# serval-uni-lu/moeva2-ijcai22-replication

Measured on AMD Instinct MI355X. Metric: candidate fitness evals/sec (whole node) + attack wall-clock per 1k states, higher is better.
Workload: dtype f64; 1 GPU; rq1.botnet.static; states=387, states_per_gpu=387, pop_size=203, n_offsprings=100, n_gen=1000, norm=2, history=reduced, classifier_dtype=f32 (MFMA), crossover=two_point, genes_stored=312, schedule=per-phase kernel chain

## Files before the change

include/moeva_mi355x.h:

```cpp
#ifndef MOEVA_MI355X_H
#define MOEVA_MI355X_H

#include <stdint.h>

#ifdef __cplusplus
extern "C" {
#endif

enum {
  MV_OK = 0,
  MV_ERR_ARG = 1,
  MV_ERR_HIP = 2,
  MV_ERR_STATE = 3,
};

enum { MV_GENE_REAL = 0, MV_GENE_INT = 1, MV_GENE_OHE = 2 };

enum {
  MV_OP_DIFF = 1,
  MV_OP_RATIO_SAFE = 2,
  MV_OP_ABS_SUMDIFF = 3,
  MV_OP_LCLD_INSTALL = 4,
  MV_OP_LCLD_TERM = 5,
  MV_OP_ABS_RATIO = 6,
// ... 84 lines not shown
  const double* ml_scale;
  const double* ml_min;
  int32_t norm;
} mv_objcalc_desc;
typedef struct mv_objcalc mv_objcalc;
int mv_objcalc_create(int32_t device, const mv_objcalc_desc* desc, mv_objcalc** out);
void mv_objcalc_destroy(mv_objcalc* o);
int mv_objcalc_run(mv_objcalc* o, mv_engine* constraints, mv_mlp* classifier, int32_t B,
                   int32_t n, const double* x_init, const double* x, int32_t minimize_class,
                   double* obj, int32_t* range_bad, void* stream);
int mv_objcalc_score(mv_objcalc* o, int32_t B, int32_t n, const double* x_init, const double* x,
                     const double* G, int32_t C, const double* proba, int32_t n_out,
                     int32_t minimize_class, double* obj, int32_t* range_bad, void* stream);
typedef struct mv_attack_params {
  int32_t n_gen;
  int32_t pop_size;
  int32_t n_offsprings;
  uint64_t seed;
  int32_t n_ref;
  const double* ref_points;
  double mu;
  int32_t history;
} mv_attack_params;

int mv_attack_run(mv_engine* e, const mv_attack_params* params, void* stream);
int mv_set_attack_mode(mv_engine* e, int32_t mode);
int mv_set_state_streams(mv_engine* e, int32_t enabled, int64_t first_state);
int mv_set_mlp_precision(mv_engine* e, int32_t bf16);
int mv_get_attack_time(mv_engine* e, double* ms, int32_t* whole);
int mv_attack_population(mv_engine* e, double* genes, double* F, void* stream);
int mv_attack_front(mv_engine* e, uint8_t* front, int32_t* offsets, double* X, double* Fx,
                    void* stream);
int mv_attack_history(mv_engine* e, double* hist, void* stream);
int mv_get_stored_genes(mv_engine* e, int32_t* stored, int32_t* n_stored);
int mv_gene_layout(mv_engine* e, int32_t B, const double* x_init, const double* xl,
                   const double* xu, int32_t* stored, int32_t* n_stored);
int mv_set_gene_layout(mv_engine* e, const int32_t* stored, int32_t V);
int mv_set_profiling(mv_engine* e, int32_t enabled);
int mv_get_kernel_times(mv_engine* e, double* vary_ms, double* mlp_ms, double* survive_ms,
                        int32_t* n_generations);
int mv_get_phase_times(mv_engine* e, double* ms, int32_t* n_generations);
int mv_get_row_kernel(mv_engine* e, int32_t* kind);
int mv_get_mlp_kernel(mv_engine* e, int32_t* kind);

int mv_debug_checks(int32_t* record, int32_t* compiled);
int mv_debug_survival_dump(double* out);

int mv_det_pow(int64_t n, const double* x, const double* y, double* out);

typedef struct mv_pgd_desc {
  int32_t D;
  const double* ml_scale;
  const double* ml_min;
  const int32_t* mutable_mask;
  int32_t C;
  const int32_t* op_code;
  const int32_t* op_arg;
  const double* op_karg;
  int32_t n_pool;
  const int32_t* idx_pool;
  int32_t n_ohe;
  const int32_t* ohe_offsets;
  const int32_t* ohe_feats;
  int32_t repair_install[4];
  double tol;
} mv_pgd_desc;
// ... 28 lines not shown
```

moeva2-ijcai22-replication_amd/csrc/api.cpp:

```cpp
#include <hip/hip_runtime.h>

#include <cmath>
#include <cstdio>
#include <cstdlib>
#include <algorithm>
#include <numeric>
#include <cstring>
#include <string>
#include <vector>

#include "../../include/moeva_mi355x.h"
#include "check.h"
#include "detmath.h"
#include "engine.h"
#include "kernels.h"
#include "pgd.h"
#include "rowops.h"

using namespace mv;

namespace mv {
thread_local hipEvent_t g_ev_start = nullptr, g_ev_stop = nullptr;
}

// ... 82 lines not shown
  DProblem p{};
  std::vector<void*> prob_allocs;
  bool compact = false;
  std::vector<int> stored;
  std::vector<int> layout_req;
  DProblem pc{};
  std::vector<void*> compact_allocs;
  DStates sc{};
  double* genes0c = nullptr;
  std::vector<void*> cstate_allocs;
  const DProblem& ap() const { return compact ? pc : p; }
  const DStates& as() const { return compact ? sc : s; }
  double* ag0() const { return compact ? genes0c : genes0; }
  float* W1full = nullptr;
  float* b1 = nullptr;
  int H1 = 0;
  int B = 0;
  std::vector<void*> state_allocs;
  DStates s{};
  double* genes0 = nullptr;
  std::vector<void*> attack_allocs;
  int P = 0, O = 0, S = 0, n_gen = 0, R = 0, hist_mode = 0, hist_w = 0, hist_rows = 0;
  double* pool = nullptr;
  double* poolF = nullptr;
  int* pop_slot = nullptr;
  int* free_slot = nullptr;
  int* parents = nullptr;
  bool has_plan = false;
  int4* plan_hdr = nullptr;
  int* plan_mw = nullptr;
  double* plan_mu = nullptr;
  double *ideal = nullptr, *worst = nullptr, *extreme = nullptr;
  int* has_ext = nullptr;
  double* ref = nullptr;
  std::vector<double> ref_host;
  double* hist = nullptr;
  unsigned char* front_scr = nullptr;
  int* off_scr = nullptr;
  bool attack_ready = false;
  bool has_model = false;
  long long* d_phase = nullptr;
  long long* d_gphase = nullptr;
  bool gphase_mlp = false;
  size_t gphase_n = 0;
  unsigned long long* dom_g = nullptr;
  size_t dom_stride = 0;
  float* xml = nullptr;
  size_t xml_cap = 0;
  hipError_t ensure_xml(size_t rows) {
    const size_t need = rows * (size_t)p.Dm4;
    if (need <= xml_cap) return hipSuccess;
    if (xml) (void)hipFree(xml);
    xml = nullptr;
    xml_cap = 0;
    hipError_t e = dalloc(&xml, need);
    if (e == hipSuccess) xml_cap = need;
    return e;
  }
  hipStream_t streams[MAX_GROUPS] = {};
  hipEvent_t ev_fork = nullptr;
  hipEvent_t ev_join[MAX_GROUPS] = {};
  hipError_t ensure_streams(int n) {
    hipError_t err = hipSuccess;
    if (!ev_fork) err = hipEventCreateWithFlags(&ev_fork, hipEventDisableTiming);
    for (int q = 1; q < n && err == hipSuccess; ++q) {
      if (!streams[q]) err = hipStreamCreateWithFlags(&streams[q], hipStreamNonBlocking);
// ... 280 lines not shown

int mv_engine_create(int32_t device, const mv_problem_desc* pd, const mv_model_desc* md,
                     mv_engine** out) {
  if (!pd || !out) return fail(MV_ERR_ARG, "null argument");
  *out = nullptr;
  const int D = pd->D, V = pd->V, Dm = pd->Dm, C = pd->C;
  if (D <= 0 || V <= 0 || Dm <= 0 || C < 0) return fail(MV_ERR_ARG, "bad problem sizes");
  if (pd->D * 4 * 8 > 160 * 1024) return fail(MV_ERR_ARG, "D too large");
  if (md && (md->n_layers < 2 || md->n_layers > MAX_LAYERS))
    return fail(MV_ERR_ARG, "classifier must have 2..6 Dense layers");
  if (md) {
    if (md->dims[0] != D) return fail(MV_ERR_ARG, "model input width != D");
    for (int l = 1; l < md->n_layers; ++l)
      if (md->dims[l] % 16 != 0 || md->dims[l] > 512 || md->dims[l] <= 0)
        return fail(MV_ERR_ARG, "hidden widths must be multiples of 16 and <= 512");
    if (md->dims[md->n_layers] < 2 || md->dims[md->n_layers] > 8)
      return fail(MV_ERR_ARG, "softmax output width must be 2..8");
  }
  for (int j = 1; j < Dm; ++j)
    if (pd->mut_feats[j] <= pd->mut_feats[j - 1]) return fail(MV_ERR_ARG, "mut_feats not ascending");
  int ns[2] = {0, 0};
  for (int g = 0; g < V; ++g) {
    const int k = pd->gene_kind[g];
    if (k < 0 || k > 2) return fail(MV_ERR_ARG, "bad gene kind");
    const int sub = ns[k == MV_GENE_REAL ? 0 : 1]++;
    if (pd->gene_feat[g] < 0 || pd->gene_feat[g] > 0x7FFF || sub > 0x7FFF)
      return fail(MV_ERR_ARG, "feature/gene index too large for the packed gene table");
  }
  if (V > VARY_MAX_V || ((Dm + 15) & ~15) > VARY_MAX_V)
    return fail(MV_ERR_ARG, "genetic length / mutable features must be <= 1024");
  HIPCHK(hipSetDevice(device));
  mv_engine* e = new mv_engine();
  e->device = device;
  HostProblem& h = e->hp;
  h.D = D;
  h.V = V;
  h.Dm = Dm;
  h.C = C;
  h.n_ohe = pd->n_ohe;
  h.n_pool = pd->n_pool;
  h.norm = pd->norm;
  h.scale_obj = pd->scale_objectives;
  h.tol = pd->tol;
  h.kind.assign(pd->gene_kind, pd->gene_kind + V);
  h.feat.assign(pd->gene_feat, pd->gene_feat + V);
  h.ohe_off.assign(pd->n_ohe + 1, 0);
  if (pd->n_ohe > 0) std::memcpy(h.ohe_off.data(), pd->ohe_offsets, (pd->n_ohe + 1) * sizeof(int));
  const int n_ohe_feats = pd->n_ohe > 0 ? pd->ohe_offsets[pd->n_ohe] : 0;
  h.ohe_feats.assign(pd->ohe_feats, pd->ohe_feats + n_ohe_feats);
  h.mut.assign(pd->mut_feats, pd->mut_feats + Dm);
  h.op_code.assign(pd->op_code, pd->op_code + C);
  h.op_arg.assign(pd->op_arg, pd->op_arg + (size_t)C * 4);
  h.op_k.assign(pd->op_karg, pd->op_karg + (size_t)C * 2);
  h.pool.assign(pd->idx_pool, pd->idx_pool + pd->n_pool);
  h.mls.assign(D, 1.0);
  h.mlm.assign(D, 0.0);
  if (pd->ml_scale) std::memcpy(h.mls.data(), pd->ml_scale, D * sizeof(double));
  if (pd->ml_min) std::memcpy(h.mlm.data(), pd->ml_min, D * sizeof(double));
  if (md) {
    e->has_model = true;
    HostModel& m = e->hm;
    m.n_layers = md->n_layers;
    for (int l = 0; l <= md->n_layers; ++l) m.dims[l] = md->dims[l];
    for (int l = 0; l < md->n_layers; ++l) {
      m.W[l].assign(md->W[l], md->W[l] + (size_t)md->dims[l] * md->dims[l + 1]);
      m.b[l].assign(md->b[l], md->b[l] + md->dims[l + 1]);
// ... 371 lines not shown
    auto A = [&](auto** dst, size_t n) {
      if (err != hipSuccess) return;
      err = dalloc(dst, n);
      if (err == hipSuccess) e->attack_allocs.push_back((void*)*dst);
    };
    e->d_gphase = nullptr;
    e->gphase_n = 0;
    e->front_scr = nullptr;
    e->off_scr = nullptr;
    A(&e->pool, (size_t)B * S * V);
    A(&e->poolF, (size_t)B * S * 3);
    A(&e->pop_slot, (size_t)B * P);
    A(&e->free_slot, (size_t)B * O);
    A(&e->parents, (size_t)B * O);
    e->plan_hdr = nullptr;
    e->plan_mw = nullptr;
    e->plan_mu = nullptr;
    if (use_plan) {
      A(&e->plan_hdr, (size_t)B * O);
      A(&e->plan_mw, (size_t)B * O * PLAN_MUT);
      A(&e->plan_mu, (size_t)B * O * PLAN_MUT);
    }
    e->has_plan = use_plan;
    e->dom_g = nullptr;
    e->dom_stride = 0;
    if (S > SURV_NLDS) {
      e->dom_stride = (size_t)S * ((S + 63) / 64);
      A(&e->dom_g, (size_t)B * e->dom_stride);
    }
    A(&e->ideal, (size_t)B * 3);
    A(&e->worst, (size_t)B * 3);
    A(&e->extreme, (size_t)B * 9);
    A(&e->has_ext, (size_t)B);
    A(&e->ref, (size_t)R * 3);
    if (prm->history) A(&e->hist, (size_t)B * hist_rows * hist_w);
    if (err != hipSuccess)
      return fail(MV_ERR_HIP, std::string("attack alloc: ") + hipGetErrorString(err));
    e->P = P;
    e->O = O;
    e->S = S;
    e->R = R;
    e->n_gen = G;
    e->hist_mode = prm->history;
    e->hist_w = hist_w;
    e->hist_rows = hist_rows;
    e->attack_ready = true;
  }
  if (realloc || e->ref_host.size() != (size_t)R * 3 ||
      std::memcmp(e->ref_host.data(), prm->ref_points, (size_t)R * 3 * sizeof(double)) != 0) {
    HIPCHK(hipDeviceSynchronize());
    e->ref_host.assign(prm->ref_points, prm->ref_points + (size_t)R * 3);
    HIPCHK(hipMemcpy(e->ref, e->ref_host.data(), (size_t)R * 3 * sizeof(double),
                     hipMemcpyHostToDevice));
  }
  hipLaunchKernelGGL(k_fill_d, dim3(64), dim3(256), 0, stream, e->ideal, (size_t)B * 3,
                     (double)INFINITY);
  hipLaunchKernelGGL(k_fill_d, dim3(64), dim3(256), 0, stream, e->worst, (size_t)B * 3,
                     (double)-INFINITY);
  hipLaunchKernelGGL(k_fill_i, dim3(64), dim3(256), 0, stream, e->has_ext, (size_t)B, 0);
  HIPCHK(hipGetLastError());
  HIPCHK(launch_init_pool(B, P, O, V, S, e->ag0(), e->pool, e->pop_slot, e->free_slot, stream));
  HIPCHK(e->ensure_xml((size_t)B * (P > O ? P : O)));
  int ngrp = B / 64;
  ngrp = ngrp > 4 ? 4 : ngrp;
  if (const char* g = std::getenv("MV_GROUPS")) ngrp = std::atoi(g);
  if (e->profiling) ngrp = 1;
  ngrp = ngrp < 1 ? 1 : (ngrp > MAX_GROUPS ? MAX_GROUPS : (ngrp > B ? B : ngrp));
  HIPCHK(e->ensure_streams(ngrp));
  hipStream_t gs[MAX_GROUPS];
  int gb0[MAX_GROUPS + 1];
  for (int q = 0; q <= ngrp; ++q) gb0[q] = (int)((long long)B * q / ngrp);
  gs[0] = stream;
  if (ngrp > 1) HIPCHK(hipEventRecord(e->ev_fork, stream));
  for (int q = 1; q < ngrp; ++q) {
    gs[q] = e->streams[q];
    HIPCHK(hipStreamWaitEvent(gs[q], e->ev_fork, 0));
  }
  const int H1 = e->H1, D = ap.D;
  const unsigned sbb = vary_offsets(ap).sb;
  const size_t Dm4 = ap.Dm4;
  auto group_rows = [&](RowsArgs r, int q, int n_per_state) {
    const size_t b0 = gb0[q];
    r.s.B = gb0[q + 1] - gb0[q];
    r.s.x_init += b0 * D;
    r.s.gl += b0 * V;
    r.s.gu += b0 * V;
    r.s.sblob += b0 * sbb;
    r.s.bias1 += b0 * H1;
    r.s.min_class += b0;
    r.total = r.s.B * n_per_state;
    r.key0 += (uint32_t)b0;
    if (r.genes_in) r.genes_in += b0 * r.in_rows * V;
    if (r.genes_out) r.genes_out += b0 * r.out_rows * V;
    if (r.parents) r.parents += b0 * O;
    if (r.out_map) r.out_map += b0 * r.n;
    if (r.plan_hdr) {
      r.plan_hdr += b0 * O;
      r.plan_mw += b0 * O * PLAN_MUT;
      r.plan_mu += b0 * O * PLAN_MUT;
    }
    if (r.F) r.F += b0 * r.out_rows * 3;
    if (r.hist) r.hist += b0 * (size_t)r.hist_rows * r.hist_w;
    r.xml += b0 * (size_t)(P > O ? P : O) * Dm4;
    return r;
  };
  auto group_surv = [&](SurvArgs s, int q) {
    const size_t b0 = gb0[q];
    s.F += b0 * S * 3;
    s.pop_slot += b0 * P;
    s.free_slot += b0 * O;
    s.pop_slot_out += b0 * P;
    s.ideal += b0 * 3;
    s.worst += b0 * 3;
    s.extreme += b0 * 9;
    s.has_extreme += b0;
    s.key0 += (uint32_t)b0;
    if (s.parents_out) s.parents_out += b0 * O;
    if (s.phase) s.phase += b0 * 32;
    if (s.dom_g) s.dom_g += b0 * s.dom_stride;
    if (s.plan_hdr) {
      s.plan_hdr += b0 * O;
      s.plan_mw += b0 * O * PLAN_MUT;
      s.plan_mu += b0 * O * PLAN_MUT;
    }
    return s;
  };
  RowsArgs ev = base_rows(e, true);
  ev.n = P;
  ev.mode = 0;
  ev.genes_in = e->pool;
  ev.in_rows = S;
  ev.out_rows = S;
  ev.F = e->poolF;
  ev.hist = prm->history ? e->hist : nullptr;
  ev.hist_rows = hist_rows;
  ev.hist_w = hist_w;
  ev.xml = e->xml;
  SurvArgs sa{};
  sa.n_survive = P;
  sa.P = P;
  sa.O = O;
  sa.F = e->poolF;
  sa.S = S;
  sa.pop_slot = e->pop_slot;
  sa.free_slot = e->free_slot;
  sa.pop_slot_out = e->pop_slot;
  sa.ref = e->ref;
  sa.R = R;
  sa.mu = prm->mu;
  sa.seed = prm->seed;
  sa.state_keys = e->state_keys;
  sa.key0 = e->key0;
  sa.ideal = e->ideal;
  sa.worst = e->worst;
  sa.extreme = e->extreme;
  sa.has_extreme = e->has_ext;
  sa.O_next = O;
  sa.dom_g = e->dom_g;
  sa.dom_stride = e->dom_stride;
  {
    int dev = 0, cus = 0;
    if (hipGetDevice(&dev) != hipSuccess ||
        hipDeviceGetAttribute(&cus, hipDeviceAttributeMultiprocessorCount, dev) != hipSuccess)
      cus = 0;
    (void)hipGetLastError();
    sa.wide = 2 * B <= cus ? 2 : B <= 2 * cus ? 1 : 0;
    if (const char* w = std::getenv("MV_SURV_WIDE")) sa.wide = std::atoi(w);
  }
  if (use_plan) {
    const VaryOff vo = vary_offsets(ap);
    sa.plan_hdr = e->plan_hdr;
    sa.plan_mw = e->plan_mw;
    sa.plan_mu = e->plan_mu;
    sa.geo = (const uint32_t*)(ap.vblob + vo.geo);
    sa.cmap = (const int*)(ap.vblob + vo.cmap);
    sa.ginfo = (const int*)(ap.vblob + vo.ginfo);
    sa.Vr = ap.Vr;
    sa.V = ap.V;
    sa.n_sub0 = ap.n_sub[0];
    sa.n_sub1 = ap.n_sub[1];
    sa.cx_prob = e->cx_prob;
    sa.cx_sbx = e->cx_kind == 1;
  }
  if (std::getenv("MV_SURV_PHASES")) {
    if (!e->d_phase) {
      HIPCHK(hipMalloc((void**)&e->d_phase, (size_t)B * 32 * sizeof(long long)));
      e->attack_allocs.push_back(e->d_phase);
    }
    sa.phase = e->d_phase;
// ... 610 lines not shown
  const DProblem& ap = e->ap();
  const int* cmap = ap.compact ? (const int*)(ap.vblob + vary_offsets(ap).cmap) : nullptr;
  HIPCHK(launch_front(e->B, e->P, ap.V, ap.Vr, e->S, cmap, e->s.gl, e->pop_slot, e->pool,
                      e->poolF, front, offsets, X, Fx, (hipStream_t)stream));
  return MV_OK;
}

int mv_gene_layout(mv_engine* e, int32_t B, const double* x_init, const double* xl,
                   const double* xu, int32_t* stored, int32_t* n_stored) {
  if (!e || B < 0 || (B > 0 && (!x_init || !xl || !xu)) || !stored || !n_stored)
    return fail(MV_ERR_ARG, "bad mv_gene_layout arguments");
  const std::vector<int> keep = B > 0 ? stored_genes(e, B, x_init, xl, xu) : std::vector<int>{};
  for (int g = 0; g < e->hp.V; ++g) stored[g] = keep.empty() ? 1 : 0;
  for (int g : keep) stored[g] = 1;
  *n_stored = keep.empty() ? e->hp.V : (int32_t)keep.size();
  return MV_OK;
}

int mv_set_gene_layout(mv_engine* e, const int32_t* stored, int32_t V) {
  if (!e) return fail(MV_ERR_ARG, "null engine");
  if (!stored) {
    e->layout_req.clear();
    return MV_OK;
  }
  if (V != e->hp.V) return fail(MV_ERR_ARG, "mv_set_gene_layout: V differs from the problem's");
  std::vector<int> keep;
  for (int g = 0; g < V; ++g)
    if (stored[g]) keep.push_back(g);
  if (keep.empty()) return fail(MV_ERR_ARG, "mv_set_gene_layout: no stored gene");
  e->layout_req = keep;
  return MV_OK;
}

int mv_get_stored_genes(mv_engine* e, int32_t* stored, int32_t* n_stored) {
  if (!e || !n_stored) return fail(MV_ERR_ARG, "null argument");
  const DProblem& ap = e->ap();
  *n_stored = ap.V;
  if (stored)
    for (int g = 0; g < ap.Vr; ++g) {
      const auto it = std::lower_bound(e->stored.begin(), e->stored.end(), g);
      stored[g] = !ap.compact || (it != e->stored.end() && *it == g);
    }
  return MV_OK;
}

int mv_attack_history(mv_engine* e, double* hist, void* stream) {
  if (!e || !e->attack_ready || !e->hist_mode) return fail(MV_ERR_STATE, "no history recorded");
  if (!hist) return fail(MV_ERR_ARG, "null hist");
  if (!on_device(hist, e->device))
    return fail(MV_ERR_ARG, "mv_attack_history: hist lives on another device than the engine");
  HIPCHK(hipSetDevice(e->device));
  HIPCHK(hipMemcpyAsync(hist, e->hist, (size_t)e->B * e->hist_rows * e->hist_w * sizeof(double),
                        hipMemcpyDefault, (hipStream_t)stream));
  return MV_OK;
}

struct mv_pgd {
  int device = 0;
  PgdArgs a{};
  std::vector<void*> allocs;
  ~mv_pgd() {
    (void)hipSetDevice(device);
    for (void* x : allocs) (void)hipFree(x);
  }
};

// ... 172 lines not shown
```

moeva2-ijcai22-replication_amd/csrc/engine.h:

```cpp
#pragma once
#include <hip/hip_runtime.h>
#include <stdint.h>

#ifndef MV_CLOCKS
#define MV_CLOCKS 0
#endif

namespace mv {

constexpr int MAX_LAYERS = 6;
constexpr int EVAL_TR = 32;
constexpr int EVAL_T = 256;
#ifndef MV_VARY_T
#define MV_VARY_T 256
#endif
constexpr int VARY_T = MV_VARY_T;
constexpr int VARY_W = VARY_T / 64;
#ifndef MV_CONS_T
#define MV_CONS_T 256
#endif
constexpr int CONS_T = MV_CONS_T;
constexpr int CONS_W = CONS_T / 64;
constexpr int VARY_ROWS_MAX = 32;
constexpr int VARY_MAX_V = 1024;
// ... 123 lines not shown
  double mu;
  uint64_t seed;
  int gen;
  uint32_t stream_key;
  int state_keys;
  uint32_t key0;
  double* ideal;
  double* worst;
  double* extreme;
  int* has_extreme;
  int* survivors;
  int* rank;
  int* order;
  int* n_ranked;
  int* niche;
  double* dist;
  double* nadir;
  int* parents_out;
  int O_next;
  int sel_gen;
  long long* phase;
  unsigned long long* dom_g;
  size_t dom_stride;
  int4* plan_hdr;
  int* plan_mw;
  double* plan_mu;
  const uint32_t* geo;
  const int* cmap;
  const int* ginfo;
  int Vr, V, n_sub0, n_sub1;
  double cx_prob;
  int cx_sbx;
  int wide;
};

struct MlpArgs {
  int n_layers;
  int dims[MAX_LAYERS + 1];
  const float* W[MAX_LAYERS];
  const float* bias[MAX_LAYERS];
  int D4;
  int n;
  const double* x;
  double* proba;
};

struct ObjArgs {
  long total;
  int n;
  int D, C, n_ohe, n_out, cls, norm;
  const double* x;
  const double* x_init;
  const double* mm_scale;
  const double* mm_min;
  const int* ohe_off;
  const int* ohe_feat;
  const double* G;
  const double* proba;
  double* obj;
  int* range_bad;
};

}
```

moeva2-ijcai22-replication_amd/csrc/survival.h:

```cpp
#pragma once
#include <limits.h>

#include "check.h"
#include "draws.h"
#include "engine.h"
#ifdef MV_CHECKS
namespace mv {
static __device__ int g_surv_dump_owner;
static __device__ double g_surv_dump[SURV_DUMP_N];
}
#endif
#include "philox.h"
#include "wave.h"

namespace mv {

constexpr int SURV_TMAX = 1024;
#ifndef MV_ASSOC_UNROLL
#define MV_ASSOC_UNROLL 1
#endif

struct SurvLds {
  double* F;
  const double* ref;
// ... 455 lines not shown
  L.cur = (unsigned long long*)(smem + o.cur);
  L.I = (int*)(smem + o.I);
  L.pos = (int*)(smem + o.pos);
  L.front_of = (int*)(smem + o.front_of);
  L.slot = (int*)(smem + o.slot);
  L.niche = (int*)(smem + o.niche);
  L.memb = (int*)(smem + o.memb);
  L.key = (int*)(smem + o.key);
  L.surv = (int*)(smem + o.surv);
  L.sel = (int*)(smem + o.sel);
  L.fstart = (int*)(smem + o.fstart);
  L.count = (int*)(smem + o.count);
  L.remain = (int*)(smem + o.remain);
  L.csr_off = (int*)(smem + o.csr_off);
  L.csr = (int*)(smem + o.csr);
  L.cand = (int*)(smem + o.cand);
  L.ckey = (int*)(smem + o.ckey);
  L.iscal = (int*)(smem + o.iscal);
  L.sortk = (unsigned long long*)(smem + o.sortk);
  L.perm = (int*)(smem + o.perm);
  L.dmin = (unsigned long long*)(smem + o.dmin);
  L.lround = (int*)(smem + o.lround);
  double* ideal = L.scal;
  double* worst = L.scal + 3;
  double* wpop = L.scal + 6;
  double* wfront = L.wsc + (tid >> 6) * 16;
  double* nadir = wfront + 3;
  double* ext = wfront + 6;
  double* pext = L.scal + 24;
  const int has_ext = a.has_extreme[b] != 0;
  const double pre_ideal = tid < 3 ? a.ideal[(size_t)b * 3 + tid] : 0.0;
  const double pre_worst = tid < 3 ? a.worst[(size_t)b * 3 + tid] : 0.0;
  const bool slot_mode = a.pop_slot != nullptr;
#define PHASE(k) \
  if (MV_CLOCKS && a.phase && tid == 0) a.phase[(size_t)b * 32 + (k)] = clock64();
  PHASE(0)

  for (int m = tid; m < N; m += T) {
    int s = m;
    const double* src;
    if (slot_mode) {
      s = m < a.P ? a.pop_slot[(size_t)b * a.P + m] : a.free_slot[(size_t)b * a.O + (m - a.P)];
      s = MV_IDX(s, a.S, CK_SURV_SLOT);
      src = a.F + ((size_t)b * a.S + s) * 3;
    } else {
      src = a.F + ((size_t)b * N + m) * 3;
    }
    const double f0 = src[0], f1 = src[1], f2 = src[2];
    L.F[m * 3 + 0] = f0;
    L.F[m * 3 + 1] = f1;
    L.F[m * 3 + 2] = f2;
    L.slot[m] = s;
    L.front_of[m] = -1;
    L.sel[m] = 0;
  }
  for (int m = N + tid; m < NW * 64; m += T) {
    L.F[m * 3 + 0] = __builtin_nan("");
    L.F[m * 3 + 1] = __builtin_nan("");
    L.F[m * 3 + 2] = __builtin_nan("");
  }
  if (tid < 9) pext[tid] = a.extreme[(size_t)b * 9 + tid];
  if (tid == 0) L.iscal[14] = 0;
  for (int q = tid; q < NW; q += T) {
    L.ranked[q] = 0ull;
    L.cur[q] = 0ull;
  }
  __syncthreads();
  PHASE(1)

  if (wave == 0) {
    double mn[3], mx[3], wp[3];
    for (int k = 0; k < 3; ++k) {
      mn[k] = __builtin_inf();
      mx[k] = -__builtin_inf();
      wp[k] = -__builtin_inf();
    }
    for (int m = lane; m < N; m += 64)
      for (int k = 0; k < 3; ++k) {
        const double v = L.F[m * 3 + k];
        mn[k] = min_prop(mn[k], v);
        mx[k] = max_prop(mx[k], v);
        wp[k] = max_prop(wp[k], v);
      }
    for (int r = lane; r < R; r += 64)
      for (int k = 0; k < 3; ++k) {
        const double v = L.ref[r * 3 + k];
        mn[k] = min_prop(mn[k], v);
        mx[k] = max_prop(mx[k], v);
      }
    for (int k = 0; k < 3; ++k) {
      mn[k] = wred_min(mn[k]);
      mx[k] = wred_max(mx[k]);
      wp[k] = wred_max(wp[k]);
    }
    if (lane < 3) {
      const int k = lane;
      double vmn = mn[0], vmx = mx[0], vwp = wp[0];
      if (k == 1) {
        vmn = mn[1];
        vmx = mx[1];
        vwp = wp[1];
      } else if (k == 2) {
        vmn = mn[2];
        vmx = mx[2];
        vwp = wp[2];
      }
      ideal[k] = min_prop(pre_ideal, vmn);
      worst[k] = max_prop(pre_worst, vmx);
      wpop[k] = vwp;
    }
  }
  PHASE(11)

  if (NWMAX * 64 > SURV_NLDS) {
    const int n_b = NW * (NW + 1) / 2;
    for (;;) {
      int t = 0;
      if (lane == 0) t = atomicAdd(&L.iscal[14], 1);
      t = __builtin_amdgcn_readfirstlane(t);
      if (t >= n_b) break;
      int qi = 0, rem = t;
      while (rem >= NW - qi) {
        rem -= NW - qi;
        ++qi;
      }
      const int qj = qi + rem;
      const int i = qi * 64 + lane;
      const double fi0 = L.F[i * 3 + 0], fi1 = L.F[i * 3 + 1], fi2 = L.F[i * 3 + 2];
      const int j0 = qj * 64;
      const double* fj = L.F + j0 * 3;
      unsigned mlo = 0u, mhi = 0u;
      unsigned long long acc = 0ull;
      DomRow<0, 64, unsigned long long>::run(fi0, fi1, fi2, fj, mlo, mhi, acc, lane);
      const unsigned long long mine = ((unsigned long long)mhi << 32) | mlo;
      if (j0 + lane < N) L.dom[(size_t)qi * N + j0 + lane] = mine;
      if (qi != qj && i < N) L.dom[(size_t)qj * N + i] = acc;
    }
  } else {
    unsigned short* dom16 = (unsigned short*)L.dom;
    const int n_q = NW * (NW + 1) * 2;
    for (;;) {
      int t = 0;
      if (lane == 0) t = atomicAdd(&L.iscal[14], 1);
      t = __builtin_amdgcn_readfirstlane(t);
      if (t >= n_q) break;
      const int qq = t & 3;
      int qi = 0, rem = t >> 2;
      while (rem >= NW - qi) {
        rem -= NW - qi;
        ++qi;
      }
      const int qj = qi + rem;
      const int i = qi * 64 + lane;
      const double fi0 = L.F[i * 3 + 0], fi1 = L.F[i * 3 + 1], fi2 = L.F[i * 3 + 2];
      const int j0 = qj * 64 + qq * 16;
      const double* fj = L.F + j0 * 3;
      unsigned mlo = 0u, mhi = 0u, acc = 0u;
      DomRow<0, 16, unsigned>::run(fi0, fi1, fi2, fj, mlo, mhi, acc, lane);
      const unsigned long long mine = ((unsigned long long)mhi << 32) | mlo;
      if (lane < 16 && j0 + lane < N)
        L.dom[(size_t)qi * N + j0 + lane] = mine;
      if (qi != qj && i < N) dom16[((size_t)qj * N + i) * 4 + qq] = (unsigned short)acc;
    }
  }
  __syncthreads();
  PHASE(2)

  int* wsum = L.iscal + 16;
  int n0 = block_compact<T>(
      N,
      [&](int j) {
        for (int q = 0; q < NW; ++q)
          if (L.dom[(size_t)q * N + j]) return false;
        return true;
      },
      L.I, 0, wsum);
  for (int k = tid; k < n0; k += T) {
    const int j = L.I[k];
    L.pos[j] = k;
    L.front_of[j] = 0;
    atomicOr(&L.ranked[j >> 6], 1ull << (j & 63));
    atomicOr(&L.cur[j >> 6], 1ull << (j & 63));
  }
  if (tid == 0) {
    L.fstart[0] = 0;
// ... 175 lines not shown
        for (int k = 0; k < 3; ++k) Mc[i][k] = M[i][k];
      bool ok = lu_solve3(Mc, plane);
      double nd[3];
      if (ok) {
        double icp[3];
        for (int k = 0; k < 3; ++k) {
          icp[k] = 1.0 / plane[k];
          nd[k] = ideal[k] + icp[k];
        }
        bool close = true, small = false;
        for (int i = 0; i < 3; ++i) {
          const double mp = (M[i][0] * plane[0] + M[i][1] * plane[1]) + M[i][2] * plane[2];
          close = close && (fabs(mp - 1.0) <= 1e-8 + 1e-5 * 1.0);
          small = small || (icp[i] <= 1e-6);
        }
        if (!close || small) {
          ok = false;
        } else {
          for (int k = 0; k < 3; ++k)
            if (nd[k] > worst[k]) nd[k] = worst[k];
        }
      }
      if (!ok)
        for (int k = 0; k < 3; ++k) nd[k] = wpop[k];
      for (int k = 0; k < 3; ++k) {
        if (nd[k] - ideal[k] <= 1e-6) nd[k] = wfront[k];
        nadir[k] = nd[k];
      }
    }
    wave_sync();
    PHASE(26)
  }
  PHASE(4)

  {
    const double nv = 1.0 / sqrt(3.0);
    const double asp = a.mu * (1.0 / 3.0);
    for (int r = tid; r < RN; r += T) {
      double res[3];
      if (r < R) {
        double l[3];
        for (int k = 0; k < 3; ++k) l[k] = (L.ref[r * 3 + k] - ideal[k]) / (nadir[k] - ideal[k]);
        const double dot = (l[0] * nv + l[1] * nv) + l[2] * nv;
        double inter[3];
        if (fabs(dot) > 1e-6) {
          const double d = ((1.0 * nv + 0.0 * nv) + 0.0 * nv) / dot;
          for (int k = 0; k < 3; ++k) inter[k] = 0.0 + l[k] * d;
        } else {
          const double q0 = l[0] - 1.0, q1 = l[1] - 0.0, q2 = l[2] - 0.0;
          const double t = (q0 * nv + q1 * nv) + q2 * nv;
          for (int k = 0; k < 3; ++k) inter[k] = l[k] - t * nv;
        }
        for (int k = 0; k < 3; ++k) res[k] = asp + (inter[k] - asp);
        if (!(res[0] > 0.0 && res[1] > 0.0 && res[2] > 0.0)) {
          for (int k = 0; k < 3; ++k)
            if (res[k] < 0.0) res[k] = 0.0;
          const double s = (res[0] + res[1]) + res[2];
          for (int k = 0; k < 3; ++k) res[k] = res[k] / s;
        }
      } else {
        for (int k = 0; k < 3; ++k) res[k] = (k == r - R) ? 1.0 : 0.0;
      }
      const double nrm = sqrt((res[0] * res[0] + res[1] * res[1]) + res[2] * res[2]);
      for (int k = 0; k < 3; ++k) L.U[r * 3 + k] = res[k] / nrm;
      L.Uf[r] = make_double4(L.U[r * 3], L.U[r * 3 + 1], L.U[r * 3 + 2], 0.0);
    }
    if (tid == 0) L.iscal[15] = 0;
    __syncthreads();
  }
  PHASE(5)

  {
    double den[3];
    for (int k = 0; k < 3; ++k) {
      den[k] = nadir[k] - ideal[k];
      if (den[k] == 0.0) den[k] = 1e-12;
    }
    const int nh = RN >> 1;
    for (int v = tid; v < 2 * n_ranked; v += T) {
      const int p = v >> 1, hf = v & 1;
      const int jb = hf ? nh : 0;
      const bool odd = hf && (RN & 1);
      const int m = L.I[p];
      double Nn[3];
      for (int k = 0; k < 3; ++k) Nn[k] = (L.F[m * 3 + k] - ideal[k]) / den[k];
      if (Nn[0] == 0.0 && Nn[1] == 0.0 && Nn[2] == 0.0 && !signbit(Nn[0]) && !signbit(Nn[1]) &&
          !signbit(Nn[2])) {
        if (!hf) {
          L.niche[p] = 0;
          L.dist[p] = 0.0;
        }
        continue;
      }
      const double nn = fma(Nn[0], Nn[0], fma(Nn[1], Nn[1], Nn[2] * Nn[2]));
      const double4* Ud = L.Uf;
      auto d2f = [&](int j) {
        const double4 u = Ud[j];
        const double sp = fma(Nn[0], u.x, fma(Nn[1], u.y, Nn[2] * u.z));
        return fma(-sp, sp, nn);
      };
      double b0 = __builtin_inf(), b1 = b0, b2 = b0, b3 = b0;
      const int n4 = nh >> 2;
      if (nn < __builtin_inf()) {
#pragma unroll MV_ASSOC_UNROLL
        for (int k = 0; k < n4; ++k) {
          const int j = jb + 4 * k;
          b0 = __builtin_fmin(b0, d2f(j));
          b1 = __builtin_fmin(b1, d2f(j + 1));
          b2 = __builtin_fmin(b2, d2f(j + 2));
          b3 = __builtin_fmin(b3, d2f(j + 3));
        }
        for (int j = jb + 4 * n4; j < jb + nh; ++j) b0 = __builtin_fmin(b0, d2f(j));
        if (odd) b0 = __builtin_fmin(b0, d2f(RN - 1));
// ... 223 lines not shown
      int r = b0;
      int t = b0;
      for (; t + 4 <= b1; t += 4) {
        const int m0 = bucket[t], m1 = bucket[t + 1], m2 = bucket[t + 2], m3 = bucket[t + 3];
        r += (sk[m0] < kp ? 1 : 0) + (sk[m1] < kp ? 1 : 0) + (sk[m2] < kp ? 1 : 0) +
             (sk[m3] < kp ? 1 : 0);
      }
      for (; t < b1; ++t) r += sk[bucket[t]] < kp ? 1 : 0;
      if (r < n_rem) L.surv[until + r] = fs + p;
    }
    for (int p = tid; p < until; p += T) L.surv[p] = p;
    n_out = a.n_survive;
  } else {
    for (int p = tid; p < n_ranked; p += T) L.surv[p] = p;
    n_out = n_ranked;
  }
  __syncthreads();
  PHASE(7)
  uint32_t* pgeo = (uint32_t*)(smem + o.ptab);
  int* pcmap = (int*)(pgeo + a.Vr + 1);
  int* pginfo = pcmap + a.Vr;
  if (plan) {
    const int nw = plan_tab_words(a.Vr, a.V);
    for (int k = tid; k < nw; k += T) {
      const int v = k <= a.Vr ? (int)a.geo[k]
                              : (k < 2 * a.Vr + 1 ? a.cmap[k - a.Vr - 1] : a.ginfo[k - 2 * a.Vr - 1]);
      pgeo[k] = (uint32_t)v;
    }
  }

  for (int k = tid; k < N; k += T) L.memb[k] = 0;
  __syncthreads();
  for (int k = tid; k < n_out; k += T) {
    const int m = L.I[L.surv[k]];
    L.memb[m] = 1;
    L.sel[k] = L.slot[m];
    if (slot_mode)
      a.pop_slot_out[(size_t)b * a.n_survive + k] = L.slot[m];
    else
      a.survivors[(size_t)b * a.n_survive + k] = m;
  }
  if (!slot_mode)
    for (int k = n_out + tid; k < a.n_survive; k += T)
      a.survivors[(size_t)b * a.n_survive + k] = -1;
  if (a.rank)
    for (int m = tid; m < N; m += T) a.rank[(size_t)b * N + m] = L.front_of[m];
  if (a.order)
    for (int p = tid; p < N; p += T) a.order[(size_t)b * N + p] = p < n_ranked ? L.I[p] : -1;
  if (a.niche)
    for (int p = tid; p < N; p += T) a.niche[(size_t)b * N + p] = p < n_ranked ? L.niche[p] : -1;
  if (a.dist)
    for (int p = tid; p < N; p += T)
      a.dist[(size_t)b * N + p] = p < n_ranked ? L.dist[p] : 0.0;
  if (tid == 0) {
    if (a.n_ranked) a.n_ranked[b] = n_ranked;
    for (int k = 0; k < 3; ++k) {
      a.ideal[(size_t)b * 3 + k] = ideal[k];
      a.worst[(size_t)b * 3 + k] = worst[k];
      if (a.nadir) a.nadir[(size_t)b * 3 + k] = nadir[k];
    }
    for (int k = 0; k < 9; ++k) a.extreme[(size_t)b * 9 + k] = ext[k];
    a.has_extreme[b] = 1;
  }
  __syncthreads();
  if (slot_mode && N > a.n_survive) {
    const int nfree = block_compact<T>(N, [&](int m) { return L.memb[m] == 0; }, L.key, 0, wsum);
#ifdef MV_CHECKS
    if (nfree != N - n_out) {
      if (tid == 0) chk_fail(CK_SURV_DUP, (long long)gen * 4096 + b, nfree);
      __shared__ int s_own;
      if (tid == 0) s_own = atomicCAS(&g_surv_dump_owner, 0, 1) == 0;
      __syncthreads();
      if (s_own) {
        double* d = g_surv_dump;
        for (int m = tid; m < N; m += T)
          for (int k = 0; k < 3; ++k)
            d[SURV_DUMP_HEAD + m * 3 + k] = a.F[((size_t)b * a.S + L.slot[m]) * 3 + k];
        if (tid < 3) {
          d[4 + tid] = pre_ideal;
          d[7 + tid] = pre_worst;
        }
        if (tid < 9) d[10 + tid] = pext[tid];
        if (tid == 0) {
          d[1] = gen;
          d[2] = b;
          d[3] = N;
          d[19] = has_ext;
          d[20] = a.n_survive;
          d[21] = __longlong_as_double((long long)a.seed);
          d[0] = 1.0;
        }
      }
    }
#endif
    for (int k = tid; k < nfree; k += T)
// ... 24 lines not shown
```

moeva2-ijcai22-replication_amd/moeva2_amd/_native.py:

```python
from __future__ import annotations

import ctypes as C
import os
from dataclasses import dataclass
from typing import List, Optional, Sequence

import numpy as np

PKG_ROOT = os.path.dirname(os.path.dirname(os.path.abspath(__file__)))
LIB_PATH = os.environ.get("MOEVA_MI355X_LIB", os.path.join(PKG_ROOT, "lib", "libmoeva_mi355x.so"))

MV_GENE_REAL, MV_GENE_INT, MV_GENE_OHE = 0, 1, 2
OP = dict(DIFF=1, RATIO_SAFE=2, ABS_SUMDIFF=3, LCLD_INSTALL=4, LCLD_TERM=5, ABS_RATIO=6,
          MONTHDIFF=7, RATIO_MASKED=8, XOR_AUG=9,
          TF_INSTALL_MIN=10, TF_HINGE_DIFF=11, TF_TERM_MIN=12, TF_RATIO_ALPHA_NEG=13,
          TF_RATIO_ALPHA_ZERO=14, TF_ABS_SUMDIFF_OFF=15)

EXPORTED = [
    "mv_last_error", "mv_device_count", "mv_engine_create", "mv_engine_destroy",
    "mv_set_states", "mv_evaluate", "mv_decode", "mv_constraints", "mv_survive", "mv_select_parents",
    "mv_variation", "mv_attack_run", "mv_attack_population", "mv_attack_front",
    "mv_attack_history",
    "mv_set_profiling", "mv_get_kernel_times", "mv_get_phase_times", "mv_get_row_kernel",
    "mv_get_mlp_kernel", "mv_set_attack_mode",
    "mv_set_crossover", "mv_set_mlp_precision",
    "mv_get_attack_time", "mv_mlp_create", "mv_mlp_destroy",
    "mv_mlp_predict", "mv_objcalc_create", "mv_objcalc_destroy", "mv_objcalc_run",
    "mv_objcalc_score", "mv_det_pow", "mv_debug_checks", "mv_set_state_streams",
    "mv_debug_survival_dump", "mv_get_stored_genes", "mv_gene_layout", "mv_set_gene_layout",
    "mv_pgd_create", "mv_pgd_destroy", "mv_pgd_grad", "mv_pgd_run", "mv_pgd_repair",
]

_i32p = C.POINTER(C.c_int32)
_f64p = C.POINTER(C.c_double)
_f32p = C.POINTER(C.c_float)


class ProblemDesc(C.Structure):
    _fields_ = [
        ("D", C.c_int32), ("V", C.c_int32), ("Dm", C.c_int32), ("C", C.c_int32),
        ("n_ohe", C.c_int32), ("gene_kind", _i32p), ("gene_feat", _i32p),
        ("ohe_offsets", _i32p), ("ohe_feats", _i32p), ("mut_feats", _i32p),
        ("ml_scale", _f64p), ("ml_min", _f64p), ("op_code", _i32p), ("op_arg", _i32p),
        ("op_karg", _f64p), ("n_pool", C.c_int32), ("idx_pool", _i32p), ("tol", C.c_double),
        ("norm", C.c_int32), ("scale_objectives", C.c_int32),
    ]


class ModelDesc(C.Structure):
    _fields_ = [("n_layers", C.c_int32), ("dims", _i32p), ("W", C.POINTER(_f32p)),
                ("b", C.POINTER(_f32p))]


class AttackParams(C.Structure):
    _fields_ = [("n_gen", C.c_int32), ("pop_size", C.c_int32), ("n_offsprings", C.c_int32),
# ... 27 lines not shown
class NativeError(RuntimeError):
    pass


_LIB = None


def lib():
    global _LIB
    if _LIB is None:
        if not os.path.exists(LIB_PATH):
            raise NativeError(
                f"{LIB_PATH} not found: build it with `make -C moeva2-ijcai22-replication_amd/csrc`"
                " (or __graft_entry__.build())")
        L = C.CDLL(LIB_PATH)
        L.mv_last_error.restype = C.c_char_p
        vp = C.c_void_p
        sig = {
            "mv_device_count": [_i32p],
            "mv_engine_create": [C.c_int32, C.POINTER(ProblemDesc), C.POINTER(ModelDesc),
                                 C.POINTER(vp)],
            "mv_set_states": [vp, C.c_int32, _f64p, _f64p, _f64p, _i32p, vp],
            "mv_evaluate": [vp, C.c_int32, vp, vp, vp, vp],
            "mv_decode": [vp, C.c_int32, vp, vp, vp],
            "mv_constraints": [vp, C.c_int32, vp, vp, vp],
            "mv_survive": [C.c_int32, C.c_int32, C.c_int32, vp, C.c_int32, vp, C.c_double,
                           C.c_uint64, C.c_int32, vp, vp, vp, vp, vp, vp, vp, vp, vp, vp, vp, vp],
            "mv_select_parents": [C.c_int32, C.c_int32, C.c_int32, C.c_uint64, C.c_int32, vp, vp],
            "mv_variation": [vp, C.c_int32, C.c_int32, C.c_uint64, C.c_int32, vp, vp, vp, vp],
            "mv_attack_run": [vp, C.POINTER(AttackParams), vp],
            "mv_attack_population": [vp, vp, vp, vp],
            "mv_attack_front": [vp, vp, vp, vp, vp, vp],
            "mv_attack_history": [vp, vp, vp],
            "mv_set_profiling": [vp, C.c_int32],
            "mv_get_kernel_times": [vp, _f64p, _f64p, _f64p, _i32p],
            "mv_get_phase_times": [vp, _f64p, _i32p],
            "mv_get_row_kernel": [vp, _i32p],
            "mv_get_mlp_kernel": [vp, _i32p],
            "mv_set_attack_mode": [vp, C.c_int32],
            "mv_set_crossover": [vp, C.c_int32, C.c_double, C.c_double],
            "mv_set_mlp_precision": [vp, C.c_int32],
            "mv_get_attack_time": [vp, _f64p, _i32p],
            "mv_mlp_create": [C.c_int32, C.POINTER(ModelDesc), C.POINTER(vp)],
            "mv_mlp_predict": [vp, C.c_int32, vp, vp, vp],
            "mv_objcalc_create": [C.c_int32, C.POINTER(ObjCalcDesc), C.POINTER(vp)],
            "mv_objcalc_run": [vp, vp, vp, C.c_int32, C.c_int32, vp, vp, C.c_int32, vp, vp, vp],
            "mv_objcalc_score": [vp, C.c_int32, C.c_int32, vp, vp, vp, C.c_int32, vp, C.c_int32,
                                 C.c_int32, vp, vp, vp],
            "mv_det_pow": [C.c_int64, _f64p, _f64p, _f64p],
            "mv_debug_checks": [_i32p, _i32p],
            "mv_set_state_streams": [vp, C.c_int32, C.c_int64],
            "mv_debug_survival_dump": [_f64p],
            "mv_get_stored_genes": [vp, _i32p, _i32p],
            "mv_gene_layout": [vp, C.c_int32, _f64p, _f64p, _f64p, _i32p, _i32p],
            "mv_set_gene_layout": [vp, _i32p, C.c_int32],
            "mv_pgd_create": [C.c_int32, C.POINTER(PgdDesc), C.POINTER(ModelDesc), C.POINTER(vp)],
            "mv_pgd_grad": [vp, C.c_int32, vp, vp, C.c_int32, C.c_int32, vp, vp, vp],
            "mv_pgd_run": [vp, C.POINTER(PgdParams), C.c_int32, vp, vp, vp, vp],
            "mv_pgd_repair": [vp, C.c_int32, vp, vp],
        }
        for name, args in sig.items():
            try:
                fn = getattr(L, name)
            except AttributeError:
                continue
            fn.argtypes = args
# ... 177 lines not shown
        check(lib().mv_decode(self._h, genes.shape[1], _ptr(genes), _ptr(x), _stream(stream)))

    def constraints(self, x, G, stream=None):
        check(lib().mv_constraints(self._h, x.shape[0], _ptr(x), _ptr(G), _stream(stream)))

    def variation(self, P, O, seed, gen, pop, parents, off, stream=None):
        check(lib().mv_variation(self._h, P, O, seed, gen, _ptr(pop), _ptr(parents), _ptr(off),
                                 _stream(stream)))

    def attack_run(self, n_gen, pop_size, n_offsprings, seed, ref_points, mu=0.05, history=0,
                   stream=None):
        ref = _arr(ref_points, np.float64)
        self._ref_keep = ref
        prm = AttackParams(n_gen, pop_size, n_offsprings, seed, ref.shape[0],
                           ref.ctypes.data_as(_f64p), mu, history)
        check(lib().mv_attack_run(self._h, C.byref(prm), _stream(stream)))

    def attack_population(self, genes=None, F=None, stream=None):
        check(lib().mv_attack_population(self._h, _ptr(genes), _ptr(F), _stream(stream)))

    def attack_front(self, front=None, offsets=None, X=None, Fx=None, stream=None):
        check(lib().mv_attack_front(self._h, _ptr(front), _ptr(offsets), _ptr(X), _ptr(Fx),
                                    _stream(stream)))

    def attack_history(self, hist, stream=None, host=False):
        if host:
            if hist.is_cuda or not hist.is_contiguous():
                raise ValueError("attack_history(host=True): a contiguous host tensor")
            p = C.c_void_p(hist.data_ptr())
        else:
            p = _ptr(hist)
        check(lib().mv_attack_history(self._h, p, _stream(stream)))

    def set_profiling(self, on: bool):
        check(lib().mv_set_profiling(self._h, int(on)))

    def set_crossover(self, kind: str = "two_point", eta: float = 30.0, prob: float = 0.9):
        check(lib().mv_set_crossover(self._h, {"two_point": 0, "sbx": 1}[kind], float(eta),
                                     float(prob)))

    def set_state_streams(self, enabled: bool, first_state: int = 0):
        check(lib().mv_set_state_streams(self._h, 1 if enabled else 0, int(first_state)))
        self.state_streams = (bool(enabled), int(first_state))

    def stored_genes(self) -> np.ndarray:
        st = np.zeros(self.prog.V, np.int32)
        n = C.c_int32(0)
        check(lib().mv_get_stored_genes(self._h, st.ctypes.data_as(_i32p), C.byref(n)))
        return st.astype(bool)

    def gene_layout(self, x_init, xl, xu) -> np.ndarray:
        x_init, xl, xu = (_arr(a, np.float64) for a in (x_init, xl, xu))
        st = np.zeros(self.prog.V, np.int32)
        n = C.c_int32(0)
        check(lib().mv_gene_layout(self._h, x_init.shape[0], x_init.ctypes.data_as(_f64p),
                                   xl.ctypes.data_as(_f64p), xu.ctypes.data_as(_f64p),
                                   st.ctypes.data_as(_i32p), C.byref(n)))
        return st.astype(bool)

    def set_gene_layout(self, stored=None):
        if stored is None:
            check(lib().mv_set_gene_layout(self._h, None, 0))
            return
        st = np.ascontiguousarray(np.asarray(stored, bool), np.int32)
        check(lib().mv_set_gene_layout(self._h, st.ctypes.data_as(_i32p), int(st.shape[0])))

# ... 215 lines not shown
```

Measured before the change: 255.8 million evals/s.

## Carry survival dominance and niche association across generations when unchanged

NSGA-III survival state now persists across generations. When the previous generation's survivors all formed a single nondominated front, the dominance tiles among the carried parents are zeroed instead of recomputed. When ideal and nadir points are bit-identical to the previous generation, reference-direction niche and distance for surviving parents are reloaded from per-slot buffers, so only offspring are re-associated. This adds per-slot global buffers, more complex tile indexing and a debug counter API, and it relies on the exact-equality conditions holding to keep results unchanged.

```diff
diff --git a/include/moeva_mi355x.h b/include/moeva_mi355x.h
--- a/include/moeva_mi355x.h
+++ b/include/moeva_mi355x.h
@@ -140,6 +140,7 @@
 int mv_attack_front(mv_engine* e, uint8_t* front, int32_t* offsets, double* X, double* Fx,
                     void* stream);
 int mv_attack_history(mv_engine* e, double* hist, void* stream);
+int mv_get_survival_carry(mv_engine* e, int32_t* dom_skipped, int32_t* assoc_reused);
 int mv_get_stored_genes(mv_engine* e, int32_t* stored, int32_t* n_stored);
 int mv_gene_layout(mv_engine* e, int32_t B, const double* x_init, const double* xl,
                    const double* xu, int32_t* stored, int32_t* n_stored);
diff --git a/moeva2-ijcai22-replication_amd/csrc/api.cpp b/moeva2-ijcai22-replication_amd/csrc/api.cpp
--- a/moeva2-ijcai22-replication_amd/csrc/api.cpp
+++ b/moeva2-ijcai22-replication_amd/csrc/api.cpp
@@ -138,6 +138,12 @@
   double* plan_mu = nullptr;
   double *ideal = nullptr, *worst = nullptr, *extreme = nullptr;
   int* has_ext = nullptr;
+  bool surv_carry = true;
+  int* carry_flag = nullptr;
+  unsigned long long* carry_bits = nullptr;
+  int* slot_niche = nullptr;
+  double* slot_dist = nullptr;
+  int* carry_cnt = nullptr;
   double* ref = nullptr;
   std::vector<double> ref_host;
   double* hist = nullptr;
@@ -484,6 +490,7 @@
   HIPCHK(hipSetDevice(device));
   mv_engine* e = new mv_engine();
   e->device = device;
+  if (const char* c = std::getenv("MV_SURV_CARRY")) e->surv_carry = c[0] != '0';
   HostProblem& h = e->hp;
   h.D = D;
   h.V = V;
@@ -921,6 +928,11 @@
     A(&e->worst, (size_t)B * 3);
     A(&e->extreme, (size_t)B * 9);
     A(&e->has_ext, (size_t)B);
+    A(&e->carry_flag, (size_t)B * 2);
+    A(&e->carry_bits, (size_t)B * 6);
+    A(&e->slot_niche, (size_t)B * S);
+    A(&e->slot_dist, (size_t)B * S);
+    A(&e->carry_cnt, (size_t)B * 2);
     A(&e->ref, (size_t)R * 3);
     if (prm->history) A(&e->hist, (size_t)B * hist_rows * hist_w);
     if (err != hipSuccess)
@@ -947,6 +959,8 @@
   hipLaunchKernelGGL(k_fill_d, dim3(64), dim3(256), 0, stream, e->worst, (size_t)B * 3,
                      (double)-INFINITY);
   hipLaunchKernelGGL(k_fill_i, dim3(64), dim3(256), 0, stream, e->has_ext, (size_t)B, 0);
+  hipLaunchKernelGGL(k_fill_i, dim3(64), dim3(256), 0, stream, e->carry_flag, (size_t)B * 2, 0);
+  hipLaunchKernelGGL(k_fill_i, dim3(64), dim3(256), 0, stream, e->carry_cnt, (size_t)B * 2, 0);
   HIPCHK(hipGetLastError());
   HIPCHK(launch_init_pool(B, P, O, V, S, e->ag0(), e->pool, e->pop_slot, e->free_slot, stream));
   HIPCHK(e->ensure_xml((size_t)B * (P > O ? P : O)));
@@ -1003,6 +1017,13 @@
     s.worst += b0 * 3;
     s.extreme += b0 * 9;
     s.has_extreme += b0;
+    if (s.carry_flag) {
+      s.carry_flag += b0 * 2;
+      s.carry_bits += b0 * 6;
+      s.slot_niche += b0 * S;
+      s.slot_dist += b0 * S;
+      s.carry_cnt += b0 * 2;
+    }
     s.key0 += (uint32_t)b0;
     if (s.parents_out) s.parents_out += b0 * O;
     if (s.phase) s.phase += b0 * 32;
@@ -1044,6 +1065,13 @@
   sa.worst = e->worst;
   sa.extreme = e->extreme;
   sa.has_extreme = e->has_ext;
+  if (e->surv_carry) {
+    sa.carry_flag = e->carry_flag;
+    sa.carry_bits = e->carry_bits;
+    sa.slot_niche = e->slot_niche;
+    sa.slot_dist = e->slot_dist;
+    sa.carry_cnt = e->carry_cnt;
+  }
   sa.O_next = O;
   sa.dom_g = e->dom_g;
   sa.dom_stride = e->dom_stride;
@@ -1720,6 +1748,24 @@
   return MV_OK;
 }
 
+int mv_get_survival_carry(mv_engine* e, int32_t* dom_skipped, int32_t* assoc_reused) {
+  if (!e || !dom_skipped || !assoc_reused) return fail(MV_ERR_ARG, "null argument");
+  if (e->B <= 0) return fail(MV_ERR_STATE, "no states bound (mv_set_states)");
+  if (!e->attack_ready) {
+    for (int b = 0; b < e->B; ++b) dom_skipped[b] = assoc_reused[b] = 0;
+    return MV_OK;
+  }
+  HIPCHK(hipSetDevice(e->device));
+  std::vector<int> c((size_t)e->B * 2);
+  HIPCHK(hipDeviceSynchronize());
+  HIPCHK(hipMemcpy(c.data(), e->carry_cnt, c.size() * sizeof(int), hipMemcpyDeviceToHost));
+  for (int b = 0; b < e->B; ++b) {
+    dom_skipped[b] = c[(size_t)b * 2];
+    assoc_reused[b] = c[(size_t)b * 2 + 1];
+  }
+  return MV_OK;
+}
+
 int mv_get_stored_genes(mv_engine* e, int32_t* stored, int32_t* n_stored) {
   if (!e || !n_stored) return fail(MV_ERR_ARG, "null argument");
   const DProblem& ap = e->ap();
diff --git a/moeva2-ijcai22-replication_amd/csrc/engine.h b/moeva2-ijcai22-replication_amd/csrc/engine.h
--- a/moeva2-ijcai22-replication_amd/csrc/engine.h
+++ b/moeva2-ijcai22-replication_amd/csrc/engine.h
@@ -179,6 +179,11 @@
   double cx_prob;
   int cx_sbx;
   int wide;
+  int* carry_flag;
+  unsigned long long* carry_bits;
+  int* slot_niche;
+  double* slot_dist;
+  int* carry_cnt;
 };
 
 struct MlpArgs {
diff --git a/moeva2-ijcai22-replication_amd/csrc/survival.h b/moeva2-ijcai22-replication_amd/csrc/survival.h
--- a/moeva2-ijcai22-replication_amd/csrc/survival.h
+++ b/moeva2-ijcai22-replication_amd/csrc/survival.h
@@ -511,6 +511,12 @@
   const double pre_ideal = tid < 3 ? a.ideal[(size_t)b * 3 + tid] : 0.0;
   const double pre_worst = tid < 3 ? a.worst[(size_t)b * 3 + tid] : 0.0;
   const bool slot_mode = a.pop_slot != nullptr;
+  const bool carry = slot_mode && a.carry_flag != nullptr;
+  const int nd_in = carry ? a.carry_flag[(size_t)b * 2] : 0;
+  const int av_in = carry ? a.carry_flag[(size_t)b * 2 + 1] : 0;
+  unsigned long long* pbits = (unsigned long long*)(L.scal + 12);
+  const int nbi = nd_in ? a.P >> 6 : 0;
+  const int njq = NWMAX * 64 > SURV_NLDS ? 4 * nbi : (nbi ? a.P >> 4 : 0);
 #define PHASE(k) \
   if (MV_CLOCKS && a.phase && tid == 0) a.phase[(size_t)b * 32 + (k)] = clock64();
   PHASE(0)
@@ -532,6 +538,26 @@
     L.slot[m] = s;
     L.front_of[m] = -1;
     L.sel[m] = 0;
+    if (av_in && m < a.P) {
+      L.surv[m] = a.slot_niche[(size_t)b * a.S + s];
+      L.sortk[m] =
+          (unsigned long long)__double_as_longlong(a.slot_dist[(size_t)b * a.S + s]);
+    }
+  }
+  if (av_in && tid < 6) pbits[tid] = a.carry_bits[(size_t)b * 6 + tid];
+  if (nbi > 0) {
+    const int PB = nbi * 64, PQ = njq * 16;
+    for (int t = tid; t < nbi * PQ; t += T) {
+      const int q = t / PQ, j = t - q * PQ;
+      L.dom[(size_t)q * N + j] = 0ull;
+    }
+    if (NWMAX * 64 <= SURV_NLDS) {
+      unsigned short* dom16 = (unsigned short*)L.dom;
+      for (int t = tid; t < (njq - 4 * nbi) * PB; t += T) {
+        const int c = 4 * nbi + t / PB, j = t % PB;
+        dom16[((size_t)(c >> 2) * N + j) * 4 + (c & 3)] = (unsigned short)0;
+      }
+    }
   }
   for (int m = N + tid; m < NW * 64; m += T) {
     L.F[m * 3 + 0] = __builtin_nan("");
@@ -592,18 +618,19 @@
   PHASE(11)
 
   if (NWMAX * 64 > SURV_NLDS) {
-    const int n_b = NW * (NW + 1) / 2;
+    const int n_b = NW * (NW + 1) / 2 - nbi * (nbi + 1) / 2;
     for (;;) {
       int t = 0;
       if (lane == 0) t = atomicAdd(&L.iscal[14], 1);
       t = __builtin_amdgcn_readfirstlane(t);
       if (t >= n_b) break;
-      int qi = 0, rem = t;
-      while (rem >= NW - qi) {
-        rem -= NW - qi;
+      int qi = 0, rem = t, c0 = nbi;
+      while (rem >= NW - c0) {
+        rem -= NW - c0;
         ++qi;
-      }
-      const int qj = qi + rem;
+        c0 = qi < nbi ? nbi : qi;
+      }
+      const int qj = c0 + rem;
       const int i = qi * 64 + lane;
       const double fi0 = L.F[i * 3 + 0], fi1 = L.F[i * 3 + 1], fi2 = L.F[i * 3 + 2];
       const int j0 = qj * 64;
@@ -617,19 +644,20 @@
     }
   } else {
     unsigned short* dom16 = (unsigned short*)L.dom;
-    const int n_q = NW * (NW + 1) * 2;
+    const int n_q = NW * (NW + 1) * 2 - (nbi * njq - 2 * nbi * (nbi - 1));
     for (;;) {
       int t = 0;
       if (lane == 0) t = atomicAdd(&L.iscal[14], 1);
       t = __builtin_amdgcn_readfirstlane(t);
       if (t >= n_q) break;
-      const int qq = t & 3;
-      int qi = 0, rem = t >> 2;
-      while (rem >= NW - qi) {
-        rem -= NW - qi;
+      int qi = 0, rem = t, c0 = njq;
+      while (rem >= 4 * NW - c0) {
+        rem -= 4 * NW - c0;
         ++qi;
-      }
-      const int qj = qi + rem;
+        c0 = qi < nbi ? njq : 4 * qi;
+      }
+      const int qq = (c0 + rem) & 3;
+      const int qj = (c0 + rem) >> 2;
       const int i = qi * 64 + lane;
       const double fi0 = L.F[i * 3 + 0], fi1 = L.F[i * 3 + 1], fi2 = L.F[i * 3 + 2];
       const int j0 = qj * 64 + qq * 16;
@@ -871,6 +899,15 @@
     PHASE(26)
   }
   PHASE(4)
+  bool reuse = false;
+  if (av_in) {
+    int eq = 1;
+    for (int k = 0; k < 3; ++k) {
+      eq &= (unsigned long long)__double_as_longlong(ideal[k]) == pbits[k] ? 1 : 0;
+      eq &= (unsigned long long)__double_as_longlong(nadir[k]) == pbits[3 + k] ? 1 : 0;
+    }
+    reuse = __builtin_amdgcn_readfirstlane(eq) != 0;
+  }
 
   {
     const double nv = 1.0 / sqrt(3.0);
@@ -904,7 +941,10 @@
       for (int k = 0; k < 3; ++k) L.U[r * 3 + k] = res[k] / nrm;
       L.Uf[r] = make_double4(L.U[r * 3], L.U[r * 3 + 1], L.U[r * 3 + 2], 0.0);
     }
-    if (tid == 0) L.iscal[15] = 0;
+    if (tid == 0) {
+      L.iscal[15] = 0;
+      L.iscal[13] = 0;
+    }
     __syncthreads();
   }
   PHASE(5)
@@ -916,8 +956,22 @@
       if (den[k] == 0.0) den[k] = 1e-12;
     }
     const int nh = RN >> 1;
-    for (int v = tid; v < 2 * n_ranked; v += T) {
-      const int p = v >> 1, hf = v & 1;
+    int n_assoc = n_ranked;
+    if (reuse) {
+      for (int p = tid; p < n_ranked; p += T) {
+        const int m = L.I[p];
+        if (m < a.P) {
+          L.niche[p] = L.surv[m];
+          L.dist[p] = __longlong_as_double((long long)L.sortk[m]);
+        } else {
+          L.memb[atomicAdd(&L.iscal[13], 1)] = p;
+        }
+      }
+      __syncthreads();
+      n_assoc = L.iscal[13];
+    }
+    for (int v = tid; v < 2 * n_assoc; v += T) {
+      const int p = reuse ? L.memb[v >> 1] : v >> 1, hf = v & 1;
       const int jb = hf ? nh : 0;
       const bool odd = hf && (RN & 1);
       const int m = L.I[p];
@@ -1207,9 +1261,14 @@
   for (int k = tid; k < N; k += T) L.memb[k] = 0;
   __syncthreads();
   for (int k = tid; k < n_out; k += T) {
-    const int m = L.I[L.surv[k]];
+    const int p = L.surv[k];
+    const int m = L.I[p];
     L.memb[m] = 1;
     L.sel[k] = L.slot[m];
+    if (carry) {
+      a.slot_niche[(size_t)b * a.S + L.slot[m]] = L.niche[p];
+      a.slot_dist[(size_t)b * a.S + L.slot[m]] = L.dist[p];
+    }
     if (slot_mode)
       a.pop_slot_out[(size_t)b * a.n_survive + k] = L.slot[m];
     else
@@ -1236,6 +1295,16 @@
     }
     for (int k = 0; k < 9; ++k) a.extreme[(size_t)b * 9 + k] = ext[k];
     a.has_extreme[b] = 1;
+    if (carry) {
+      a.carry_flag[(size_t)b * 2] = nf == 1 && n_out == a.n_survive ? 1 : 0;
+      a.carry_flag[(size_t)b * 2 + 1] = 1;
+      for (int k = 0; k < 3; ++k) {
+        a.carry_bits[(size_t)b * 6 + k] = (unsigned long long)__double_as_longlong(ideal[k]);
+        a.carry_bits[(size_t)b * 6 + 3 + k] = (unsigned long long)__double_as_longlong(nadir[k]);
+      }
+      if (nbi > 0) a.carry_cnt[(size_t)b * 2] += 1;
+      if (reuse) a.carry_cnt[(size_t)b * 2 + 1] += 1;
+    }
   }
   __syncthreads();
   if (slot_mode && N > a.n_survive) {
diff --git a/moeva2-ijcai22-replication_amd/moeva2_amd/_native.py b/moeva2-ijcai22-replication_amd/moeva2_amd/_native.py
--- a/moeva2-ijcai22-replication_amd/moeva2_amd/_native.py
+++ b/moeva2-ijcai22-replication_amd/moeva2_amd/_native.py
@@ -20,7 +20,7 @@
     "mv_last_error", "mv_device_count", "mv_engine_create", "mv_engine_destroy",
     "mv_set_states", "mv_evaluate", "mv_decode", "mv_constraints", "mv_survive", "mv_select_parents",
     "mv_variation", "mv_attack_run", "mv_attack_population", "mv_attack_front",
-    "mv_attack_history",
+    "mv_attack_history", "mv_get_survival_carry",
     "mv_set_profiling", "mv_get_kernel_times", "mv_get_phase_times", "mv_get_row_kernel",
     "mv_get_mlp_kernel", "mv_set_attack_mode",
     "mv_set_crossover", "mv_set_mlp_precision",
@@ -114,6 +114,7 @@
             "mv_attack_population": [vp, vp, vp, vp],
             "mv_attack_front": [vp, vp, vp, vp, vp, vp],
             "mv_attack_history": [vp, vp, vp],
+            "mv_get_survival_carry": [vp, _i32p, _i32p],
             "mv_set_profiling": [vp, C.c_int32],
             "mv_get_kernel_times": [vp, _f64p, _f64p, _f64p, _i32p],
             "mv_get_phase_times": [vp, _f64p, _i32p],
@@ -357,6 +358,13 @@
             p = _ptr(hist)
         check(lib().mv_attack_history(self._h, p, _stream(stream)))
 
+    def survival_carry(self):
+        dom = np.zeros(self.B, np.int32)
+        assoc = np.zeros(self.B, np.int32)
+        check(lib().mv_get_survival_carry(self._h, dom.ctypes.data_as(_i32p),
+                                          assoc.ctypes.data_as(_i32p)))
+        return dom, assoc
+
     def set_profiling(self, on: bool):
         check(lib().mv_set_profiling(self._h, int(on)))
 
```

Result: faster. 267.0 million evals/s (median of 6 runs) (+4.4%).
